# xionghuichen/mopo

Measured on AMD Instinct MI355X. Metric: model-rollout transitions/s (halfcheetah-mixed), higher is better.
Workload: dtype f32 (exact f32 operands: each split into 3 round-to-nearest bf16 parts with x0+x1+x2 == x for 2^-100 <= |x| < 2^127; 6 bf16 MFMA products, the 3 dropped ones <= 2^-23 |x w| in total; f32 accumulate; held to the fp32 parity tolerances); rollout actor: the same exact bf16x6 split; 1 GPU; C2 rollout: E=7 (5 elites), H=200 smv, obs=17, act=6, rollout_batch=50000 per GPU, horizon=5, penalty_coeff=1, learned-var penalty, env pool 101000 rows; rollout_batch_per_gpu=50000, horizon=5, parallelism=dp1

## Files before the change

### include/mopo_hip.h

```cpp
#ifndef MOPO_HIP_H
#define MOPO_HIP_H
#include <stdint.h>

#ifdef __cplusplus
extern "C" {
#endif

const char* mopo_last_error(void);
int mopo_version(void);

typedef struct mopo_bnn_s* mopo_bnn_t;

int mopo_bnn_create(mopo_bnn_t* out, int E, int obs_dim, int act_dim, int hidden, int smv, int dtype);
int mopo_bnn_device_hidden(int hidden, int dtype, int wide);
int mopo_bnn_destroy(mopo_bnn_t h);
int mopo_bnn_set_params(mopo_bnn_t h, const float* const* h_arrays, int n_arrays);
int mopo_bnn_predict(mopo_bnn_t h, const void* d_inputs, int inputs_f64, int64_t B,
                     float* d_mean, float* d_var, void* stream);
int64_t mopo_bnn_packed_bytes(mopo_bnn_t h);
int mopo_bnn_packed_copy(mopo_bnn_t h, int to_handle, void* d_buf, int64_t nbytes, void* stream);

enum { MOPO_TERM_NONE = 0, MOPO_TERM_HALFCHEETAH = 0, MOPO_TERM_WALKER2D = 1, MOPO_TERM_HOPPER = 2,
       MOPO_TERM_ANT = 3, MOPO_TERM_HUMANOID = 4, MOPO_TERM_KINDS = 5 };

typedef struct {
  const void* d_obs;
  int obs_f64;
  const float* d_act;
  int64_t B;
  const double* d_noise_sel;
  const int64_t* d_model_inds;
  int deterministic;
  float penalty_coeff;
  int penalty_learned_var;
  int term_kind;
  double* d_next_obs;
  double* d_rewards;
// ... 158 lines not shown
```

### mopo_amd/_lib.py

```python
import ctypes as C
import os

_HERE = os.path.dirname(os.path.abspath(__file__))
LIB_PATH = os.path.join(_HERE, 'libmopo_hip.so')

c_void_p, c_int, c_i64, c_u64, c_u32, c_float, c_double = (
    C.c_void_p, C.c_int, C.c_int64, C.c_uint64, C.c_uint32, C.c_float, C.c_double)


class FakeEnvArgs(C.Structure):
    _fields_ = [('d_obs', c_void_p), ('obs_f64', c_int), ('d_act', c_void_p), ('B', c_i64),
                ('d_noise_sel', c_void_p), ('d_model_inds', c_void_p), ('deterministic', c_int),
                ('penalty_coeff', c_float), ('penalty_learned_var', c_int), ('term_kind', c_int),
                ('d_next_obs', c_void_p), ('d_rewards', c_void_p), ('d_terminals', c_void_p),
                ('d_penalty', c_void_p), ('d_unpenalized', c_void_p), ('d_info_mean', c_void_p),
                ('d_info_std', c_void_p), ('d_log_prob', c_void_p), ('d_dev', c_void_p),
                ('d_ens_mean', c_void_p), ('d_ens_var', c_void_p)]


class PoolDesc(C.Structure):
    _fields_ = [('d_obs', c_void_p), ('d_act', c_void_p), ('d_rew', c_void_p), ('d_term', c_void_p),
                ('d_next_obs', c_void_p), ('d_state', c_void_p), ('max_size', c_i64)]


class RolloutArgs(C.Structure):
    _fields_ = [('d_env_obs', c_void_p), ('env_size', c_i64), ('d_start_idx', c_void_p),
                ('d_pi_params', c_void_p), ('pi_hidden', c_int), ('d_elites', c_void_p),
                ('n_elites', c_int), ('B', c_i64), ('horizon', c_int), ('penalty_coeff', c_float),
                ('term_kind', c_int), ('seed', c_u64), ('epoch', c_u32), ('uid_offset', c_i64),
                ('d_eps_act', c_void_p), ('d_eps_obs', c_void_p), ('d_model_inds', c_void_p),
                ('d_steps', c_void_p), ('penalty_learned_var', c_int), ('deterministic', c_int),
                ('rollout_random', c_int), ('d_act_uniform', c_void_p), ('actor_dtype', c_int)]


class EvalArgs(C.Structure):
    _fields_ = [('policy_deterministic', c_int), ('d_return', c_void_p), ('d_pen_return', c_void_p),
                ('d_pen_sum', c_void_p), ('d_length', c_void_p), ('d_terminated', c_void_p), ('d_stats', c_void_p)]


SIGNATURES = {
    'mopo_last_error': (C.c_char_p, []),
    'mopo_version': (c_int, []),
    'mopo_bnn_create': (c_int, [C.POINTER(c_void_p), c_int, c_int, c_int, c_int, c_int, c_int]),
    'mopo_bnn_destroy': (c_int, [c_void_p]),
    'mopo_bnn_set_params': (c_int, [c_void_p, C.POINTER(c_void_p), c_int]),
    'mopo_actor_device_hidden': (c_int, [c_int, c_int]),
    'mopo_bnn_device_hidden': (c_int, [c_int, c_int, c_int]),
    'mopo_bnn_predict': (c_int, [c_void_p, c_void_p, c_int, c_i64, c_void_p, c_void_p, c_void_p]),
    'mopo_bnn_packed_bytes': (c_i64, [c_void_p]),
    'mopo_bnn_packed_copy': (c_int, [c_void_p, c_int, c_void_p, c_i64, c_void_p]),
    'mopo_fakeenv_step': (c_int, [c_void_p, C.POINTER(FakeEnvArgs), c_void_p]),
    'mopo_sac_param_count': (c_i64, [c_int, c_int, c_int]),
    'mopo_actor_forward': (c_int, [c_void_p, c_int, c_int, c_int, c_void_p, c_int, c_i64, c_void_p,
                                   c_u64, c_u32, c_void_p, c_void_p, c_void_p]),
    'mopo_actor_forward_dtype': (c_int, [c_void_p, c_int, c_int, c_int, c_void_p, c_int, c_i64, c_void_p,
                                         c_u64, c_u32, c_void_p, c_void_p, c_int, c_void_p]),
    'mopo_pool_add': (c_int, [C.POINTER(PoolDesc), c_int, c_int, c_void_p, c_void_p, c_void_p, c_void_p,
                              c_void_p, c_i64, c_void_p]),
    'mopo_pool_gather': (c_int, [C.POINTER(PoolDesc), c_int, c_int, c_void_p, c_i64, c_void_p, c_void_p,
                                 c_void_p, c_void_p, c_void_p, c_i64, c_void_p]),
    'mopo_pool_random_indices': (c_int, [C.POINTER(PoolDesc), c_i64, c_u64, c_u32, c_void_p, c_void_p]),
    'mopo_pool_staged_block_bytes': (c_i64, [c_int, c_int, c_i64]),
    'mopo_pool_add_blocks': (c_int, [C.POINTER(PoolDesc), c_int, c_int, c_void_p, c_i64, c_int, c_i64, c_void_p,
                                     c_void_p]),
    'mopo_rollout_run_staged_steps': (c_int, [c_void_p, C.POINTER(RolloutArgs), C.POINTER(PoolDesc), c_int, c_int,
                                              c_void_p]),
    'mopo_bnn_train_create': (c_int, [C.POINTER(c_void_p), c_int, c_int, c_int, c_int, c_int, c_int, C.c_float]),
    'mopo_bnn_train_destroy': (c_int, [c_void_p]),
    'mopo_bnn_train_set_params': (c_int, [c_void_p, C.POINTER(c_void_p)]),
    'mopo_bnn_train_get_params': (c_int, [c_void_p, C.POINTER(c_void_p)]),
# ... 86 lines not shown
```

### mopo_amd/csrc/bnn_api.hip

```cpp
#include "mlp_tile.h"

#include <cmath>
#include <cstring>
#include <memory>
#include <string>
#include <vector>

using namespace mopo;

extern "C" int mopo_bnn_create(mopo_bnn_t* out, int E, int obs_dim, int act_dim, int hidden, int smv,
                               int dtype) {
  MOPO_REQUIRE(out != nullptr, "mopo_bnn_create: out is NULL");
  MOPO_REQUIRE(E >= 1 && E <= 256, "mopo_bnn_create: num_networks must be in [1, 256]");
  MOPO_REQUIRE(obs_dim >= 1 && act_dim >= 1, "mopo_bnn_create: bad obs/act dims");
  MOPO_REQUIRE(dtype >= 0 && dtype <= 4,
               "mopo_bnn_create: dtype must be 0 (fp32), 1 (bf16), 2 (bf16x3), 3 (bf16x6) or 4 (f16x3)");
  auto h = std::make_unique<Bnn>();
  h->E = E; h->O = obs_dim; h->A = act_dim; h->H = hidden; h->smv = smv; h->dtype = dtype;
  BnnDev& d = h->dev;
  d.E = E; d.O = obs_dim; d.A = act_dim; d.IN = obs_dim + act_dim; d.H = hidden; d.D = obs_dim + 1;
  if (d.IN > 16 * MAX_IN_KG || d.D > 32) {
    return fail("mopo_bnn_create: obs_dim + act_dim must be <= 64 and obs_dim <= 31 (got obs_dim " +
                std::to_string(obs_dim) + ", act_dim " + std::to_string(act_dim) + ")");
  }
// ... 14 lines not shown
  if (dtype == 3 && d.NB2 > 16) {
    return fail("mopo_bnn_create: bf16x6 supports hidden sizes <= 256 (use f16x3 or fp32)");
  }
  const int form = bnn_form_blocks(hidden, dtype, wide);
  if (form < 0) {
    if (dtype == DT_BF16 || dtype == DT_BF16X3)
      return fail("mopo_bnn_create: bf16 and bf16x3 run hidden sizes up to 64, 193..208 and 385..416 only (got " +
                  std::to_string(hidden) + "; fp32, bf16x6 and f16x3 run every hidden size up to 256)");
    return fail("mopo_bnn_create: no kernel for hidden size " + std::to_string(hidden) +
                " (every hidden size up to 256 runs in fp32, bf16x6 and f16x3, 385..400 in fp32 and f16x3; a wide "
                "model's bf16x6 / f16x3 stop at 208)");
  }
  h->HD = bnn_device_hidden(hidden, dtype, wide);
  d.NBH = form;
  d.NB2 = (d.NBH + 1) / 2 * 2;
  d.BS = d.NB2 * 16;
  *out = reinterpret_cast<mopo_bnn_t>(h.release());
  return 0;
}

extern "C" int mopo_bnn_device_hidden(int hidden, int dtype, int wide) {
  if (dtype < 0 || dtype > 4) return -1;
  return bnn_device_hidden(hidden, dtype, wide != 0);
}

extern "C" int mopo_bnn_destroy(mopo_bnn_t hh) {
  Bnn* h = reinterpret_cast<Bnn*>(hh);
  if (!h) return 0;
  if (h->buf) (void)hipFree(h->buf);
  if (h->bbuf) (void)hipFree(h->bbuf);
  delete h;
  return 0;
}

extern "C" int mopo_bnn_set_params(mopo_bnn_t hh, const float* const* arrs, int n) {
  Bnn* h = reinterpret_cast<Bnn*>(hh);
  MOPO_REQUIRE(h != nullptr, "mopo_bnn_set_params: NULL handle");
  MOPO_REQUIRE(n == (h->smv ? 16 : 14), "mopo_bnn_set_params: expected 16 (smv) or 14 arrays (.mat keys)");
  BnnDev& d = h->dev;
  const int E = h->E, IN = d.IN, H = h->H, D = d.D;
  const int KG0 = d.KG0, NBH = d.NBH, NBO = d.NBO;
  const int64_t hp = d.BS;
  const int64_t s_w0 = (int64_t)E * KG0 * NBH * 256, s_wh = 3LL * E * NBH * NBH * 256,
                s_whd = (int64_t)E * NBH * NBO * 256, s_b0 = E * hp, s_bh = 3 * E * hp,
                s_bhd = (int64_t)E * 3 * NBO * 16;
  const int64_t s_ws = (5LL * E + 63) / 64 * 64;
// ... 54 lines not shown
  }
  if (rc == 0) rc = pack(head.data(), head.size(), whd, H, 2 * D, NBH, NBO, 2);
  if (rc) return rc;
  {
    std::vector<float> aux((size_t)s_bhd, 0.f);
    for (int e = 0; e < E; ++e) {
      float* x = aux.data() + (size_t)e * 3 * NBO * 16;
      for (int sl = 0; sl < NBO * 16; ++sl) {
        const int c = head_col(sl, D);
        if (c < 0) continue;
        x[sl] = headb[(size_t)e * 2 * D + c];
        if (c >= D) {
          x[NBO * 16 + sl] = arrs[h->smv ? 14 : 12][c - D];
          x[2 * NBO * 16 + sl] = arrs[h->smv ? 15 : 13][c - D];
        }
      }
    }
    MOPO_HIP(hipMemcpy(bhd, aux.data(), aux.size() * sizeof(float), hipMemcpyHostToDevice));
  }
  if (h->dtype != 0 && rc == 0) {
    const int NB2 = d.NB2, KG = NB2 / 2, P = bf16_parts(h->dtype), KG0B = (KG0 + 1) / 2;
    const bool kpack = bnn_kpack(h->dtype, NB2, NBH, h->HD);
    const int64_t SLM = kpack ? (KG - 1) * P + 1 : KG * P;
    const int64_t f0 = (int64_t)E * KG0B * P * NB2, fh = 3LL * E * SLM * NB2, fd = (int64_t)E * SLM * NBO;
    if (!h->bbuf) MOPO_HIP(hipMalloc(&h->bbuf, (f0 + fh + fd) * 256 * sizeof(float)));
    h->bbuf_bytes = (f0 + fh + fd) * 256 * (int64_t)sizeof(float);
    float* b0f = reinterpret_cast<float*>(h->bbuf);
    float* bhf = b0f + f0 * 256;
    float* bdf = bhf + fh * 256;
    std::vector<float> scale_h(5 * E), inv_h(5 * E, 1.f);
    float* scale_d = nullptr;
    DevFree scale_guard{scale_d};
    if (h->dtype == DT_F16X3) MOPO_HIP(hipMalloc(&scale_d, E * sizeof(float)));
    auto member_scales = [&](const float* src, int K, int N, int layer) {
      for (int e = 0; e < E; ++e) {
        float m = 0.f;
        for (int64_t i = 0; i < (int64_t)K * N; ++i) m = std::max(m, std::fabs(src[(int64_t)e * K * N + i]));
        int ex = 0;
        if (m > 0.f && std::isfinite(m)) std::frexp(m, &ex);
        const int k = m > 0.f && std::isfinite(m) ? 15 - ex : 0;
        scale_h[layer * E + e] = std::ldexp(1.f, k);
        inv_h[layer * E + e] = std::ldexp(1.f, -k);
      }
    };
    int layer_idx = 0;
    auto packh = [&](const float* src, size_t nsrc, float* dst, int K, int N, int KGb, int NB, int perm_n,
                     bool pk = false) -> int {
      MOPO_HIP(hipMemcpy(stage, src, nsrc * sizeof(float), hipMemcpyHostToDevice));
      const int64_t mstride = (pk ? SLM : (int64_t)KGb * P) * NB;
      if (pk) {
        if (pack_frags_kpack(stage, (short*)dst, E, K, N, KGb, NB, perm_n, mstride, 0)) return -1;
        --KGb;
      }
      if (h->dtype == DT_F16X3) {
        member_scales(src, K, N, layer_idx);
        MOPO_HIP(hipMemcpy(scale_d, scale_h.data() + layer_idx * E, E * sizeof(float), hipMemcpyHostToDevice));
      }
      if (pack_frags16(stage, (short*)dst, E, K, N, KGb, NB, perm_n, P, h->dtype == DT_F16X3 ? scale_d : nullptr, mstride, 0))
        return -1;
      MOPO_HIP(hipDeviceSynchronize());
      ++layer_idx;
      return 0;
    };
    if (rc == 0) rc = packh(W[0], (size_t)E * IN * H, b0f, IN, H, KG0B, NB2, 1);
    for (int l = 0; l < 3 && rc == 0; ++l)
      rc = packh(W[1 + l], (size_t)E * H * H, bhf + (int64_t)l * E * SLM * NB2 * 256, H, H, KG, NB2, 1, kpack);
    if (rc == 0) rc = packh(head.data(), head.size(), bdf, H, 2 * D, KG, NBO, 2, kpack);
    if (rc == 0 && h->dtype == DT_F16X3)
      rc = hipMemcpy(wsc, inv_h.data(), 5 * E * sizeof(float), hipMemcpyHostToDevice) == hipSuccess ? 0
                                                                                                 : fail("bnn: scale copy");
    d.w0b = b0f; d.whb = bhf; d.whdb = bdf; d.wscale = wsc;
  }
  if (rc) return -1;
  MOPO_HIP(hipMemcpy(mu, arrs[0], IN * sizeof(float), hipMemcpyHostToDevice));
  MOPO_HIP(hipMemcpy(sg, arrs[1], IN * sizeof(float), hipMemcpyHostToDevice));
  MOPO_HIP(hipMemcpy(mx, maxlv, D * sizeof(float), hipMemcpyHostToDevice));
  MOPO_HIP(hipMemcpy(mn, minlv, D * sizeof(float), hipMemcpyHostToDevice));
  d.w0 = w0; d.wh = wh; d.whd = whd; d.b0 = b0; d.bh = bh; d.bhd = bhd;
  d.mu = mu; d.sigma = sg; d.maxlv = mx; d.minlv = mn;
  h->has_params = true;
  return 0;
}

extern "C" int mopo_bnn_predict(mopo_bnn_t hh, const void* x, int x_f64, int64_t B, float* mean,
                                float* var, void* stream) {
  Bnn* h = reinterpret_cast<Bnn*>(hh);
  MOPO_REQUIRE(h != nullptr, "mopo_bnn_predict: NULL handle");
  MOPO_REQUIRE(B >= 0 && B < (1LL << 31) / 32, "mopo_bnn_predict: batch too large");
  if (B == 0) return 0;
  MOPO_REQUIRE(x && mean && var, "mopo_bnn_predict: NULL pointer");
// ... 34 lines not shown
```

### mopo_amd/csrc/bnn_kernels.h

```cpp
#pragma once
#include "mlp_tile.h"

#include <type_traits>

#ifndef BNN_KPB
#define BNN_KPB 1
#endif
#ifndef BNN_MINB_WIDE
#define BNN_MINB_WIDE 2
#endif
#ifndef BNN_R13
#define BNN_R13 1
#endif
#ifndef BNN_FWD_WAVES
#define BNN_FWD_WAVES 4
#endif
#ifndef BNN_SPLIT_HOLD_F32
#define BNN_SPLIT_HOLD_F32 1
#endif
#ifndef BNN_SPLIT_MINB
#define BNN_SPLIT_MINB 3
#endif
#ifndef BNN_SPLIT_WAVES
#define BNN_SPLIT_WAVES 4
// ... 596 lines not shown
    layer2(w.whb + ((int64_t)l * E + e) * KG * P * NB2 * 256, hf, std::integral_constant<int, KG>{},
           w.bh + ((int64_t)l * E + e) * bs);
    to_input(lds_bias, inv_row * w.wscale[(1 + l) * E + e]);
  }
  f32x4 hd[NBO];
  layer_lds_split_f32<KG, NBO, WAVES, SLOT, P, 1, true, NBO, KH>(w.whdb + (int64_t)e * KG * P * NBO * 256, hf, hd,
                                                                 lds, wv, lane, s_in);
  const float f = inv_row * w.wscale[4 * E + e] * kNegLn2;
#pragma unroll
  for (int nb = 0; nb < NBO; ++nb) hd[nb] *= f;
  int lane_e;
  asm volatile("v_mbcnt_lo_u32_b32 %0, -1, 0\n\tv_mbcnt_hi_u32_b32 %0, -1, %0" : "=v"(lane_e));
  const int64_t row_e = (int64_t)((grp * WAVES + __builtin_amdgcn_readfirstlane(wv)) * 16 + (lane_e & 15));
  const bool ok_e = row_e < count;
  head_epilogue<NBO, MODE>(w, a, hd, e, row_e, count, g, w.bhd + (int64_t)e * 3 * NBO * 16,
                           (MODE == FWD_ROLLOUT && a.sel && ok_e) ? a.sel[row_e] : -1);
}

template <int NB2, int P, int WAVES>
constexpr int ring_minb() {
  const int b = (P == 3 ? (NB2 == 16 ? BNN_RING_MINB_X6_16 : BNN_RING_MINB_X6) : BNN_RING_MINB) * 4 / WAVES;
  return b > 0 ? b : 1;
}
template <int NB2, int NBO, int MODE, int WAVES, int P, int DEPTH, int NBU = NB2, int KG0B = 1, bool KP = false>
__global__ __launch_bounds__(WAVES * 64, (ring_minb<NB2, P, WAVES>())) void bnn_fwd_ring_kernel(const BnnDev w, const FwdArgs a) {
  static_assert(P == 1 || P == 2 || P == 3, "1: bf16, 2: f16x3, 3: bf16x6 (the exact 3-part bf16 split)");
  static_assert(DEPTH >= 3, "ring of at least 3 slots");
  constexpr bool F16 = P == 2;
  constexpr bool RBUF = true;
  constexpr int HPS = BNN_RING_HEAD_MERGE && Stage<P * NBO, WAVES>::SLOTS <= Stage<NB2, WAVES>::SLOTS ? P : 1;
  constexpr int P0 = P * KG0B;
  constexpr bool KH = NBU < NB2;
  static_assert(!KP || (P == 3 && KH), "the packed remainder is the 3-part split's, behind an odd block count");
  constexpr int KG = NB2 / 2, KGF = KP ? KG - 1 : KG;
  constexpr int SLH = KGF * P + KP, SLD = KGF * (P / HPS) + KP;
  constexpr int NS = P0 + 3 * SLH + SLD;
  constexpr int JHEAD = P0 + 3 * SLH;
  constexpr int SLOT = Stage<(NB2 > HPS * NBO ? NB2 : HPS * NBO), WAVES>::SLOTS * 256;
  constexpr int BIAS_LDS = (NB2 * 4 + 63) / 64 * 256;
  __shared__ __attribute__((aligned(16))) float lds[DEPTH * SLOT + 2 * BIAS_LDS];
  float* lds_bias0 = lds + DEPTH * SLOT;
  const int lane = threadIdx.x & 63, wv = __builtin_amdgcn_readfirstlane(threadIdx.x >> 6), m = lane & 15, g = lane >> 4;
  const int64_t count = a.d_count ? (int64_t)*a.d_count : a.B;
  const int groups = ceil_div(a.ntiles, WAVES);
  const int C = ceil_div(groups, 8);
  const int xcd = blockIdx.x & 7, jb = blockIdx.x >> 3;
  const int e = __builtin_amdgcn_readfirstlane(jb / C), grp = __builtin_amdgcn_readfirstlane(xcd * C + jb % C);
  if (grp >= groups) return;
  const int64_t row = (int64_t)(grp * WAVES + wv) * 16 + m;
  if ((int64_t)grp * WAVES * 16 >= count) return;
  const int IN = w.IN, O = w.O, E = w.E;
  const bool ok = row < count;
  auto row_max = [&](float mx) {
    mx = fmaxf(mx, __shfl_xor(mx, 16));
    return fmaxf(mx, __shfl_xor(mx, 32));
  };
// ... 60 lines not shown
    row_scale(row_max(mx0), s_in, inv_row);
  }
  wait_vm_lgkm0<0>();
  __builtin_amdgcn_sched_barrier(0);
  stage_bias<NB2 * 4, WAVES, RBUF>(w.b0 + e * bs, lds_bias0, wv, lane);
  RingRun<0, DEPTH - 1>::run([&](auto jc) { issue(jc); });

  constexpr float kNegLog2e = -1.4426950408889634f, kNegLn2 = -0.6931471805599453f;
  f32x4 acc[NB2 > NBO ? NB2 : NBO];
  float hf[KG][8];
  bf16x8 cur[P];
  const float* lds_bias = lds_bias0;
  auto bias4 = [&](int off) { return __builtin_bit_cast(f32x4, *reinterpret_cast<const bf16x8*>(lds_bias + off)); };
  constexpr bool DEF = BNN_F16Q_DEFER;
  constexpr bool FOLD = F16 && DEF && BNN_F16_FOLD;
  auto to_input = [&](float f) {
    float mx = 0.f;
#pragma unroll
    for (int c = 0; c < KG; ++c) {
      const f32x4 b0 = bias4((2 * c) * 16 + 4 * g);
      const f32x4 b1 = bias4((2 * c + 1) * 16 + 4 * g);
#pragma unroll
      for (int t = 0; t < 4; ++t) {
        const float u0 = fmaf(acc[2 * c][t], f, b0[t]);
        const float u1 = 2 * c + 1 < NBU ? fmaf(acc[2 * c + 1][t], f, b1[t]) : 0.f;
        hf[c][t] = DEF ? u0 : swish_log2(u0);
        hf[c][4 + t] = DEF || 2 * c + 1 >= NBU ? u1 : swish_log2(u1);
        if constexpr (F16) mx = fmaxf(mx, fmaxf(fabsf(hf[c][t]), fabsf(hf[c][4 + t])));
      }
    }
    if constexpr (F16) row_scale(row_max(mx), s_in, inv_row);
  };
  auto act = [&](int c, int j) {
    if ((j < 4 || 2 * c + 1 < NBU) && !(KP && c == KG - 1 && j >= 2)) {
      const float u = hf[c][j];
      hf[c][j] = FOLD ? u * __builtin_amdgcn_rcpf(fmaf(__builtin_amdgcn_exp2f(u), inv_row, inv_row)) : swish_log2(u);
    }
  };
  auto parts = [&](const float (&v)[8], auto prescaled, auto half) {
    if constexpr (F16) {
      u32x4v h4, l4;
#pragma unroll
      for (int q = 0; q < 4; ++q) {
        if (decltype(half)::value && q >= 2) {
          h4[q] = l4[q] = 0u;
          continue;
        }
// ... 27 lines not shown
  };
  auto parts_rem = [&](const float (&v)[8]) {
    if constexpr (P == 3) {
      uint32_t pr[3];
      split_bf16_pair<3>(v[0], v[1], pr);
      u32x4v bf, bh;
#pragma unroll
      for (int d = 0; d < 4; ++d) {
        bf[d] = pr[kpack_slot(2 * d).xp];
        bh[d] = d < 2 ? pr[kpack_slot(d < 2 ? 8 + 2 * d : 8).xp] : 0u;
      }
      cur[0] = __builtin_bit_cast(bf16x8, bf);
      cur[1] = __builtin_bit_cast(bf16x8, bh);
    }
  };
  auto layer = [&](auto Lc, auto& in) {
    constexpr int L = decltype(Lc)::value;
    constexpr int KGL = L == 0 ? KG0B : KG, NBL = L == 4 ? NBO : NB2, NBUL = L == 4 ? NBO : NBU;
    constexpr bool KHL = L > 0 && KH;
    constexpr bool DEFER = DEF && L > 0;
    constexpr int J0 = L == 0 ? 0 : P0 + SLH * (L - 1);
    constexpr int PPS = L == 4 ? HPS : 1, SPK = P / PPS;
    constexpr bool KPL = KP && L > 0;
    constexpr int SLL = SPK * (KPL ? KGL - 1 : KGL) + KPL;
    static_assert(SLL == (L == 0 ? P0 : L == 4 ? SLD : SLH), "the layer's share of the slice stream");
#pragma unroll
    for (int nb = 0; nb < NBL; ++nb) acc[nb] = zero4();
    if constexpr (DEFER) {
#pragma unroll
      for (int j = 0; j < 8; ++j) act(0, j);
    }
    RingRun<J0, J0 + SLL>::run([&](auto jc) {
      constexpr int J = decltype(jc)::value, s = J - J0;
      constexpr bool REM = KPL && s == SLL - 1;
      constexpr int kg = REM ? KGL - 1 : s / SPK, p0 = REM ? 0 : (s % SPK) * PPS;
      if constexpr (REM)
        parts_rem(in[kg]);
      else if constexpr (p0 == 0)
        parts(in[kg], std::integral_constant<bool, FOLD && (L > 0)>{}, std::integral_constant<bool, KHL && kg + 1 == KGL>{});
      constexpr int N = [] {
        int n = 0;
        for (int i = 1; i <= DEPTH - 2; ++i) {
          const int Jx = J + i;
          const int nf = Jx < JHEAD ? NB2 : (KP && Jx == NS - 1 ? NBO : HPS * NBO);
          n += Jx >= NS ? 0 : (nf + WAVES - 1) / WAVES;
        }
// ... 1 lines not shown
      }();
      wait_vm_lgkm0<N>();
      __builtin_amdgcn_s_barrier();
      if constexpr (s == 0 && L < 3)
        stage_bias<NB2 * 4, WAVES, RBUF>(w.bh + ((int64_t)L * E + e) * bs, lds_bias0 + ((L + 1) & 1) * BIAS_LDS, wv, lane);
      issue(std::integral_constant<int, J + DEPTH - 1>{});
      __builtin_amdgcn_sched_barrier(0);
      const float* b = lds + (J % DEPTH) * SLOT;
      auto frag = [&](int i) { return *reinterpret_cast<const bf16x8*>(b + (((i / NBUL) * NBL + i % NBUL) * 64 + lane) * 4); };
      constexpr int PF = P == 3 ? (NB2 == 16 ? BNN_RING_PF_X6_16 : BNN_RING_PF_X6) : BNN_RING_PF, NFR = REM ? NBUL : PPS * NBUL;
      bf16x8 fq[PF];
#pragma unroll
      for (int k = 0; k < PF; ++k)
        if (k < NFR) fq[k] = frag(k);
#pragma unroll
      for (int i = 0; i < NFR; ++i) {
        const int p = p0 + i / NBUL, nb = i % NBUL;
        const bf16x8 fr = fq[i % PF];
        if (i + PF < NFR) fq[i % PF] = frag(i + PF);
        if constexpr (BNN_RING_PIN) __builtin_amdgcn_sched_barrier(0x0406);
        if constexpr (REM) {
          acc[nb] = mfma_16x16x32<F16>(fr, cur[0], acc[nb]);
          acc[nb] = mfma_16x16x32<F16>(fr, cur[1], acc[nb]);
        } else {
#pragma unroll
          for (int q = P - 1 - p; q >= 0; --q)
            acc[nb] = (KHL && kg + 1 == KGL) ? mfma_16x16x16_lo<F16>(fr, cur[q], acc[nb])
                                             : mfma_16x16x32<F16>(fr, cur[q], acc[nb]);
        }
        if constexpr (DEFER && kg + 1 < KGL) {
          constexpr int V = (8 + P - 1) / P;
#pragma unroll
          for (int v = 0; v < V; ++v)
            if (V * p + v < 8 && nb == ((v + 1) * NBUL / V - 1 > 0 ? (v + 1) * NBUL / V - 1 : 0)) act(kg + 1, V * p + v);
        }
      }
    });
  };
  {
    float x1[KG0B][8];
#pragma unroll
    for (int c = 0; c < KG0B; ++c)
#pragma unroll
      for (int j = 0; j < 8; ++j) x1[c][j] = xv[c][j];
    layer(std::integral_constant<int, 0>{}, x1);
  }
  to_input(inv_row * wsc[0] * kNegLog2e);
  layer(std::integral_constant<int, 1>{}, hf);
  lds_bias = lds_bias0 + BIAS_LDS;
  to_input(inv_row * wsc[1]);
  layer(std::integral_constant<int, 2>{}, hf);
  lds_bias = lds_bias0;
  to_input(inv_row * wsc[2]);
  layer(std::integral_constant<int, 3>{}, hf);
  lds_bias = lds_bias0 + BIAS_LDS;
  to_input(inv_row * wsc[3]);
  layer(std::integral_constant<int, 4>{}, hf);
  f32x4 hd[NBO];
  const float f = inv_row * wsc[4] * kNegLn2;
#pragma unroll
  for (int nb = 0; nb < NBO; ++nb) hd[nb] = acc[nb] * f;
  int lane_e;
  asm volatile("v_mbcnt_lo_u32_b32 %0, -1, 0\n\tv_mbcnt_hi_u32_b32 %0, -1, %0" : "=v"(lane_e));
  const int64_t row_e = (int64_t)(grp * WAVES + wv) * 16 + (lane_e & 15);
  const bool ok_e = row_e < count;
  head_epilogue<NBO, MODE>(w, a, hd, e, row_e, count, g, w.bhd + (int64_t)e * 3 * NBO * 16,
                           (MODE == FWD_ROLLOUT && a.sel && ok_e) ? a.sel[row_e] : -1);
}

template <class F>
static inline void with_mode(int mode, F&& f) {
  if (mode == FWD_PREDICT) f(std::integral_constant<int, FWD_PREDICT>{});
  else f(std::integral_constant<int, FWD_ROLLOUT>{});
}

template <int NB2, int NBO, int P, int DEPTH, int KG0B = 1, bool KP = false>
static int launch_ring(const Bnn* h, int mode, FwdArgs a, hipStream_t s) {
  constexpr int WV = BNN_RING_WAVES;
  a.ntiles = (int)ceil_div((int)a.B, 16);
  if (a.ntiles == 0) return 0;
  dim3 grid(8 * ceil_div(ceil_div(a.ntiles, WV), 8) * h->E), block(64 * WV);
  constexpr int NBU = NB2 == 14 ? NB2 - 1 : NB2;
  with_mode(mode, [&](auto m) {
    hipLaunchKernelGGL((bnn_fwd_ring_kernel<NB2, NBO, decltype(m)::value, WV, P, DEPTH, NBU, KG0B, KP>), grid, block, 0, s,
                       h->dev, a);
  });
  MOPO_HIP(hipGetLastError());
  return 0;
}
template <int NB2>
static bool ring_shape(const Bnn* h) { return NB2 <= 16 && (NB2 == 14 ? h->dev.NBH == 13 : h->dev.NBH == NB2); }
static inline bool kpack_shape(const Bnn* h) { return bnn_kpack(h->dtype, h->dev.NB2, h->dev.NBH, h->HD); }
template <int NB2, int NBO, int KG0B = 1>
static int launch_ring_x6(const Bnn* h, int mode, const FwdArgs& a, hipStream_t s) {
  if constexpr (NB2 == 14)
    if (kpack_shape(h)) return launch_ring<NB2, NBO, 3, BNN_RING_DEPTH_BF16, KG0B, true>(h, mode, a, s);
  if (kpack_shape(h)) return fail("bnn bf16x6: packed-remainder weights at a shape without the packed kernel");
  return launch_ring<NB2, NBO, 3, BNN_RING_DEPTH_BF16, KG0B>(h, mode, a, s);
}

constexpr int FWD_WAVES = BNN_FWD_WAVES;

template <int KG0, int NBH, int NBO, int R, int TQ0 = 4, int TQH = 4>
static int launch_fwd_t(const Bnn* h, int mode, FwdArgs a, hipStream_t s) {
  a.ntiles = (int)ceil_div((int)a.B, 16 * R);
  if (a.ntiles == 0) return 0;
  dim3 grid(ceil_div(a.ntiles, FWD_WAVES) * h->E), block(64 * FWD_WAVES);
  with_mode(mode, [&](auto m) {
    hipLaunchKernelGGL((bnn_fwd_kernel<KG0, NBH, NBO, R, decltype(m)::value, FWD_WAVES, TQ0, TQH>), grid, block, 0, s,
                       h->dev, a);
  });
  MOPO_HIP(hipGetLastError());
  return 0;
}

}
```

### mopo_amd/csrc/bnn_pack.h

```cpp
#pragma once
#include "mlp_tile.h"

#include <algorithm>

namespace mopo {

__global__ void pack_frags_kernel(const float* __restrict__ src, float* __restrict__ dst, int E, int K,
                                  int N, int KG, int NB, int perm_k, int perm_n) {
  int64_t total = (int64_t)E * KG * NB * 256;
  for (int64_t i = blockIdx.x * (int64_t)blockDim.x + threadIdx.x; i < total;
       i += (int64_t)gridDim.x * blockDim.x) {
    int t = i & 3, lane = (i >> 2) & 63;
    int64_t f = i >> 8;
    int nb = f % NB;
    int kg = (f / NB) % KG;
    int e = f / ((int64_t)NB * KG);
    int k = kg * 16 + 4 * (lane >> 4) + t, n = nb * 16 + (lane & 15);
    if (perm_k) k = slot_feat(k, K);
    if (perm_n == 1) n = slot_feat(n, N);
    else if (perm_n == 2) n = head_col(n, N / 2);
    dst[i] = (k >= 0 && n >= 0 && k < K && n < N) ? src[((int64_t)e * K + k) * N + n] : 0.f;
  }
}

// ... 26 lines not shown
__global__ void pack_frags_kpack_kernel(const float* __restrict__ src, short* __restrict__ dst, int E, int K, int N,
                                        int KG, int NB, int perm_n, int64_t mstride) {
  int64_t total = (int64_t)E * NB * 512;
  for (int64_t i = blockIdx.x * (int64_t)blockDim.x + threadIdx.x; i < total;
       i += (int64_t)gridDim.x * blockDim.x) {
    int j = i & 7, lane = (i >> 3) & 63;
    int64_t f = i >> 9;
    int nb = f % NB;
    int e = f / NB;
    const KPackSlot sl = kpack_slot(j);
    int k = slot_feat((KG - 1) * 32 + bf16_kperm(lane >> 4, sl.k), K), n = nb * 16 + (lane & 15);
    if (perm_n == 1) n = slot_feat(n, N);
    else if (perm_n == 2) n = head_col(n, N / 2);
    short parts[3];
    split_bf16<3>((k >= 0 && n >= 0 && k < K && n < N) ? src[((int64_t)e * K + k) * N + n] : 0.f, parts);
    short v = parts[0];
#pragma unroll
    for (int q = 1; q < 3; ++q)
      if (q == sl.wp) v = parts[q];
    dst[(e * mstride + (int64_t)(KG - 1) * 3 * NB + nb) * 512 + (i & 511)] = v;
  }
}

__global__ void pack_frags_f16s_kernel(const float* __restrict__ src, short* __restrict__ dst, int E, int K, int N,
                                       int KG, int NB, int perm_k, int perm_n, const float* __restrict__ scale) {
  constexpr int P = 2;
  int64_t total = (int64_t)E * KG * P * NB * 512;
  for (int64_t i = blockIdx.x * (int64_t)blockDim.x + threadIdx.x; i < total;
       i += (int64_t)gridDim.x * blockDim.x) {
    int j = i & 7, lane = (i >> 3) & 63;
    int64_t f = i >> 9;
    int nb = f % NB;
    int p = (f / NB) % P;
    int kg = (f / ((int64_t)NB * P)) % KG;
    int e = f / ((int64_t)NB * P * KG);
    int k = kg * 32 + bf16_kperm(lane >> 4, j), n = nb * 16 + (lane & 15);
    if (perm_k) k = slot_feat(k, K);
    if (perm_n == 1) n = slot_feat(n, N);
    else if (perm_n == 2) n = head_col(n, N / 2);
    const F16Parts q = split_f16_scaled((k >= 0 && n >= 0 && k < K && n < N) ? src[((int64_t)e * K + k) * N + n] : 0.f,
                                        scale[e]);
    dst[i] = p == 0 ? q.hi : q.lo;
  }
}

__global__ void pack_bias_kernel(const float* __restrict__ src, float* __restrict__ dst, int E, int N,
// ... 19 lines not shown
  MOPO_HIP(hipGetLastError());
  return 0;
}

int pack_frags16(const float* src, short* dst, int E, int K, int N, int KG, int NB, int perm_n, int P,
                 const float* scale, int64_t mstride, hipStream_t s) {
  const dim3 grid = pack_grid((int64_t)E * KG * P * NB * 512), block(256);
  if (scale) hipLaunchKernelGGL(pack_frags_f16s_kernel, grid, block, 0, s, src, dst, E, K, N, KG, NB, 1, perm_n, scale);
  else if (P == 3) hipLaunchKernelGGL(pack_frags_bf16_kernel<3>, grid, block, 0, s, src, dst, E, K, N, KG, NB, 1, perm_n, mstride);
  else if (P == 2) hipLaunchKernelGGL(pack_frags_bf16_kernel<2>, grid, block, 0, s, src, dst, E, K, N, KG, NB, 1, perm_n, mstride);
  else hipLaunchKernelGGL(pack_frags_bf16_kernel<1>, grid, block, 0, s, src, dst, E, K, N, KG, NB, 1, perm_n, mstride);
  MOPO_HIP(hipGetLastError());
  return 0;
}

int pack_frags_kpack(const float* src, short* dst, int E, int K, int N, int KG, int NB, int perm_n, int64_t mstride,
                     hipStream_t s) {
  hipLaunchKernelGGL(pack_frags_kpack_kernel, pack_grid((int64_t)E * NB * 512), dim3(256), 0, s, src, dst, E, K, N, KG, NB,
                     perm_n, mstride);
  MOPO_HIP(hipGetLastError());
  return 0;
}

}
```

### mopo_amd/csrc/internal.h

```cpp
#pragma once
#include "common.h"
#include "../../include/mopo_hip.h"

namespace mopo {

constexpr int MAX_IN_KG = 4;
__host__ __device__ constexpr bool bnn_wide(int IN, int D) { return IN > 32 || D > 24; }

struct BnnDev {
  int E, O, A, IN, H, D;
  int KG0, NBH, NBO;
  const float* w0;
  const float* wh;
  const float* whd;
  const float* b0;
  const float* bh;
  const float* bhd;
  const float* mu;
  const float* sigma;
  const float* maxlv;
  const float* minlv;
  int BS;
  int NB2;
  const float* w0b;
  const float* whb;
  const float* whdb;
  const float* wscale;
};

enum { DT_FP32 = 0, DT_BF16 = 1, DT_BF16X3 = 2, DT_BF16X6 = 3, DT_F16X3 = 4 };
__host__ __device__ constexpr int bf16_parts(int dtype) { return dtype < 1 ? 1 : (dtype == DT_F16X3 ? 2 : dtype); }

__host__ __device__ constexpr int tail_steps(int F) { return (F & 15) == 0 ? 4 : ((F & 15) + 3) >> 2; }

__host__ __device__ constexpr bool bnn_kpack(int dtype, int NB2, int NBH, int H) {
  return dtype == DT_BF16X6 && NB2 == 14 && NBH == 13 && tail_steps(H) == 2;
}

inline int bnn_form_blocks(int hidden, int dtype, bool wide) {
  if (hidden < 1) return -1;
  const int nb = (hidden + 15) / 16;
  const bool split = dtype == 3  || dtype == 4 ;
  if (!wide && dtype != 0) {
    if (dtype != 4 && (nb == 1 || nb == 3)) return nb;
    if (dtype != 3 && nb == 26) return nb;
    if (!split) return (nb == 2 || nb == 4 || nb == 13 || nb == 25) ? nb : -1;
  }
  if (wide && dtype != 0 && !split) return -1;
  const int forms[6] = {2, 4, 8, 13, 16, 25};
  const int top = dtype == 0 ? 25 : (wide ? 13 : (dtype == 3 ? 16 : 25));
  for (int f : forms)
    if (f >= nb && f <= top) return (f == 25 && nb < 25) ? -1 : f;
  return -1;
}
inline int bnn_device_hidden(int hidden, int dtype, bool wide) {
  const int f = bnn_form_blocks(hidden, dtype, wide);
  if (f < 0) return -1;
  const int lo = (f == 8 || f == 16) ? 16 * f : 16 * (f - 1) + 1;
  return hidden > lo ? hidden : lo;
// ... 35 lines not shown
  int ntiles;
  int xcd_members;
  float* mean;
  float* var;
  uint32_t* pen_bits;
  const int32_t* sel;
  float* mean_sel;
  float* std_sel;
  float* mean_all;
  float* std_all;
  int64_t all_stride;
};

int launch_bnn_fwd(const Bnn* h, int mode, const FwdArgs& a, hipStream_t s);
int launch_bnn_fwd_widths(const Bnn* h, int mode, const FwdArgs& a, hipStream_t s);
int launch_bnn_fwd_widths16(const Bnn* h, int mode, const FwdArgs& a, hipStream_t s);
int pack_frags(const float* src, float* dst, int E, int K, int N, int KG, int NB, hipStream_t s, int perm_k = 0,
               int perm_n = 0);
int pack_bias(const float* src, float* dst, int E, int N, int NP, float mul, hipStream_t s);
int pack_frags16(const float* src, short* dst, int E, int K, int N, int KG, int NB, int perm_n, int P,
                 const float* scale, int64_t mstride, hipStream_t s);
int pack_frags_kpack(const float* src, short* dst, int E, int K, int N, int KG, int NB, int perm_n, int64_t mstride,
                     hipStream_t s);

template <class F>
__device__ __forceinline__ bool term_fn_at(int kind, const F& nobs, int O) {
  if (kind == MOPO_TERM_WALKER2D) {
    double hh = nobs(0), an = nobs(1);
    bool not_done = (hh > 0.8) && (hh < 2.0) && (an > -1.0) && (an < 1.0);
    return !not_done;
  }
  if (kind == MOPO_TERM_HOPPER) {
    bool fin = true, small = true;
    for (int d = 0; d < O; ++d) {
      double v = nobs(d);
      fin = fin && isfinite(v);
      if (d >= 1) small = small && (v < 100.0);
    }
    double hh = nobs(0), an = nobs(1);
    bool not_done = fin && small && (hh > 0.7) && (fabs(an) < 0.2);
    return !not_done;
  }
  if (kind == MOPO_TERM_ANT) {
    bool fin = true;
    for (int d = 0; d < O; ++d) fin = fin && isfinite(nobs(d));
    double x = nobs(0);
// ... 16 lines not shown
```

### mopo_amd/csrc/mlp_tile.h

```cpp
#pragma once
#include <type_traits>

#include "internal.h"

namespace mopo {

__host__ __device__ __forceinline__ int slot_feat(int slot, int F) {
  const int blk = slot >> 4, rem = F - 16 * blk;
  if (rem >= 16) return slot;
  if (rem <= 0) return -1;
  const int q = (rem + 3) >> 2, g = (slot >> 2) & 3, t = slot & 3, f = q * g + t;
  return (t < q && f < rem) ? 16 * blk + f : -1;
}

__host__ __device__ __forceinline__ int head_col(int slot, int D) {
  const int nb = slot >> 4, g = (slot >> 2) & 3, t = slot & 3, j = 4 * nb + t, Q = (D + 3) >> 2;
  if (j < Q) return g + 4 * j < D ? D + g + 4 * j : -1;
  if (j < 2 * Q) return g + 4 * (j - Q) < D ? g + 4 * (j - Q) : -1;
  return -1;
}


typedef __attribute__((address_space(3))) void* lds_void_t;

// ... 242 lines not shown

struct KPackSlot {
  int k, xp, wp;
};
constexpr int KPACK_SLOTS = 12;
__host__ __device__ constexpr KPackSlot kpack_slot(int i) {
  constexpr int XP[6] = {0, 0, 0, 1, 2, 1}, WP[6] = {0, 1, 2, 0, 0, 1};
  return {i & 1, XP[i >> 1], WP[i >> 1]};
}
constexpr bool kpack_table_ok() {
  for (int k = 0; k < 2; ++k)
    for (int p = 0; p < 3; ++p)
      for (int q = 0; q < 3; ++q) {
        int n = 0;
        for (int i = 0; i < KPACK_SLOTS; ++i) n += kpack_slot(i).k == k && kpack_slot(i).xp == p && kpack_slot(i).wp == q;
        if (n != (p + q < 3 ? 1 : 0)) return false;
      }
  for (int i = 8; i < KPACK_SLOTS; ++i)
    if (kpack_slot(i).wp != kpack_slot(i - 8).wp) return false;
  return true;
}
static_assert(kpack_table_ok(), "every product (p, q), p + q < 3, exactly once per k, and no other");

template <int KG, int NB, int WAVES, int SLOT, int P, int PS = P, bool F16 = false, int NBU = NB, bool KH = false>
__device__ __forceinline__ void layer_lds_split(const float* __restrict__ wf, const bf16x8 (&in)[P][KG],
                                                f32x4 (&acc)[NB], float* lds, int w, int lane,
                                                const float* __restrict__ bias = nullptr, float* lds_bias = nullptr) {
  static_assert(P % PS == 0, "parts per slice must divide the parts");
  constexpr int SPK = P / PS, S = KG * SPK, NF = PS * NB;
  static_assert(Stage<NF, WAVES>::SLOTS * 256 <= SLOT, "slice larger than its buffer");
#pragma unroll
  for (int nb = 0; nb < NB; ++nb) acc[nb] = zero4();
  __syncthreads();
  stage_slice<NF, WAVES>(wf, lds, w, lane);
  if (bias) stage_bias<NB * 4, WAVES>(bias, lds_bias, w, lane);
#pragma unroll
  for (int s = 0; s < S; ++s) {
    __syncthreads();
    if (s + 1 < S) stage_slice<NF, WAVES>(wf + (s + 1) * NF * 256, lds + ((s + 1) & 1) * SLOT, w, lane);
    __builtin_amdgcn_sched_barrier(0);
    const int kg = s / SPK;
    const float* b = lds + (s & 1) * SLOT;
#ifndef BNN_SPLIT_NOPF
    bf16x8 fr_next = *reinterpret_cast<const bf16x8*>(b + lane * 4);
#endif
#pragma unroll
// ... 173 lines not shown
```

Baseline: 102.2 million transitions/s.

## Pack the half-used last output block's split products into fewer MFMAs

For the bf16x6 ring kernel at the 13-block hidden shape, the last output column block only uses half its columns. The half-empty column slots now carry different weight parts of the same columns, so each k-slice issues fewer MFMAs for that block, and the two halves are summed afterwards. This needs a new weight-packing kernel, an mpack mode template parameter, and zeroing of the padded outputs. The aim is to cut wasted matrix-core work on padding columns, at the cost of a more intricate packing scheme that must still produce each split product exactly once.

```diff
diff --git a/include/mopo_hip.h b/include/mopo_hip.h
--- a/include/mopo_hip.h
+++ b/include/mopo_hip.h
@@ -13,6 +13,7 @@
 
 int mopo_bnn_create(mopo_bnn_t* out, int E, int obs_dim, int act_dim, int hidden, int smv, int dtype);
 int mopo_bnn_device_hidden(int hidden, int dtype, int wide);
+int mopo_bnn_mpack(int hidden, int dtype, int obs_dim, int act_dim);
 int mopo_bnn_destroy(mopo_bnn_t h);
 int mopo_bnn_set_params(mopo_bnn_t h, const float* const* h_arrays, int n_arrays);
 int mopo_bnn_predict(mopo_bnn_t h, const void* d_inputs, int inputs_f64, int64_t B,
diff --git a/mopo_amd/_lib.py b/mopo_amd/_lib.py
--- a/mopo_amd/_lib.py
+++ b/mopo_amd/_lib.py
@@ -46,6 +46,7 @@
     'mopo_bnn_set_params': (c_int, [c_void_p, C.POINTER(c_void_p), c_int]),
     'mopo_actor_device_hidden': (c_int, [c_int, c_int]),
     'mopo_bnn_device_hidden': (c_int, [c_int, c_int, c_int]),
+    'mopo_bnn_mpack': (c_int, [c_int, c_int, c_int, c_int]),
     'mopo_bnn_predict': (c_int, [c_void_p, c_void_p, c_int, c_i64, c_void_p, c_void_p, c_void_p]),
     'mopo_bnn_packed_bytes': (c_i64, [c_void_p]),
     'mopo_bnn_packed_copy': (c_int, [c_void_p, c_int, c_void_p, c_i64, c_void_p]),
diff --git a/mopo_amd/csrc/bnn_api.hip b/mopo_amd/csrc/bnn_api.hip
--- a/mopo_amd/csrc/bnn_api.hip
+++ b/mopo_amd/csrc/bnn_api.hip
@@ -60,6 +60,16 @@
 extern "C" int mopo_bnn_device_hidden(int hidden, int dtype, int wide) {
   if (dtype < 0 || dtype > 4) return -1;
   return bnn_device_hidden(hidden, dtype, wide != 0);
+}
+
+extern "C" int mopo_bnn_mpack(int hidden, int dtype, int obs_dim, int act_dim) {
+  if (dtype < 0 || dtype > 4 || obs_dim < 1 || act_dim < 0) return -1;
+  const int IN = obs_dim + act_dim, D = obs_dim + 1;
+  if (IN > 16 * MAX_IN_KG || D > 32) return -1;
+  const bool wide = bnn_wide(IN, D);
+  const int NBH = bnn_form_blocks(hidden, dtype, wide);
+  if (NBH < 0) return -1;
+  return bnn_mpack(dtype, (NBH + 1) / 2 * 2, NBH, bnn_device_hidden(hidden, dtype, wide), D, wide ? 4 : ceil_div(2 * D, 16));
 }
 
 extern "C" int mopo_bnn_destroy(mopo_bnn_t hh) {
@@ -160,6 +170,7 @@
     const int NB2 = d.NB2, KG = NB2 / 2, P = bf16_parts(h->dtype), KG0B = (KG0 + 1) / 2;
     const bool kpack = bnn_kpack(h->dtype, NB2, NBH, h->HD);
     const int64_t SLM = kpack ? (KG - 1) * P + 1 : KG * P;
+    const int mpack = bnn_mpack(h->dtype, NB2, NBH, h->HD, D, NBO);
     const int64_t f0 = (int64_t)E * KG0B * P * NB2, fh = 3LL * E * SLM * NB2, fd = (int64_t)E * SLM * NBO;
     if (!h->bbuf) MOPO_HIP(hipMalloc(&h->bbuf, (f0 + fh + fd) * 256 * sizeof(float)));
     h->bbuf_bytes = (f0 + fh + fd) * 256 * (int64_t)sizeof(float);
@@ -183,7 +194,7 @@
     };
     int layer_idx = 0;
     auto packh = [&](const float* src, size_t nsrc, float* dst, int K, int N, int KGb, int NB, int perm_n,
-                     bool pk = false) -> int {
+                     bool pk = false, int mpb = -1) -> int {
       MOPO_HIP(hipMemcpy(stage, src, nsrc * sizeof(float), hipMemcpyHostToDevice));
       const int64_t mstride = (pk ? SLM : (int64_t)KGb * P) * NB;
       if (pk) {
@@ -196,14 +207,16 @@
       }
       if (pack_frags16(stage, (short*)dst, E, K, N, KGb, NB, perm_n, P, h->dtype == DT_F16X3 ? scale_d : nullptr, mstride, 0))
         return -1;
+      if (mpb >= 0 && pack_frags_mpack(stage, (short*)dst, E, K, N, KGb, NB, mpb, perm_n, mstride, 0)) return -1;
       MOPO_HIP(hipDeviceSynchronize());
       ++layer_idx;
       return 0;
     };
-    if (rc == 0) rc = packh(W[0], (size_t)E * IN * H, b0f, IN, H, KG0B, NB2, 1);
+    const int mpb = mpack ? NBH - 1 : -1, mpbd = mpack == 2 ? NBO - 1 : -1;
+    if (rc == 0) rc = packh(W[0], (size_t)E * IN * H, b0f, IN, H, KG0B, NB2, 1, false, mpb);
     for (int l = 0; l < 3 && rc == 0; ++l)
-      rc = packh(W[1 + l], (size_t)E * H * H, bhf + (int64_t)l * E * SLM * NB2 * 256, H, H, KG, NB2, 1, kpack);
-    if (rc == 0) rc = packh(head.data(), head.size(), bdf, H, 2 * D, KG, NBO, 2, kpack);
+      rc = packh(W[1 + l], (size_t)E * H * H, bhf + (int64_t)l * E * SLM * NB2 * 256, H, H, KG, NB2, 1, kpack, mpb);
+    if (rc == 0) rc = packh(head.data(), head.size(), bdf, H, 2 * D, KG, NBO, 2, kpack, mpbd);
     if (rc == 0 && h->dtype == DT_F16X3)
       rc = hipMemcpy(wsc, inv_h.data(), 5 * E * sizeof(float), hipMemcpyHostToDevice) == hipSuccess ? 0
                                                                                                  : fail("bnn: scale copy");
diff --git a/mopo_amd/csrc/bnn_kernels.h b/mopo_amd/csrc/bnn_kernels.h
--- a/mopo_amd/csrc/bnn_kernels.h
+++ b/mopo_amd/csrc/bnn_kernels.h
@@ -642,7 +642,7 @@
   const int b = (P == 3 ? (NB2 == 16 ? BNN_RING_MINB_X6_16 : BNN_RING_MINB_X6) : BNN_RING_MINB) * 4 / WAVES;
   return b > 0 ? b : 1;
 }
-template <int NB2, int NBO, int MODE, int WAVES, int P, int DEPTH, int NBU = NB2, int KG0B = 1, bool KP = false>
+template <int NB2, int NBO, int MODE, int WAVES, int P, int DEPTH, int NBU = NB2, int KG0B = 1, bool KP = false, int MP = 0>
 __global__ __launch_bounds__(WAVES * 64, (ring_minb<NB2, P, WAVES>())) void bnn_fwd_ring_kernel(const BnnDev w, const FwdArgs a) {
   static_assert(P == 1 || P == 2 || P == 3, "1: bf16, 2: f16x3, 3: bf16x6 (the exact 3-part bf16 split)");
   static_assert(DEPTH >= 3, "ring of at least 3 slots");
@@ -652,6 +652,7 @@
   constexpr int P0 = P * KG0B;
   constexpr bool KH = NBU < NB2;
   static_assert(!KP || (P == 3 && KH), "the packed remainder is the 3-part split's, behind an odd block count");
+  static_assert(MP == 0 || ((MP == 1 || MP == 2) && KP), "the packed output block comes with the packed remainder");
   constexpr int KG = NB2 / 2, KGF = KP ? KG - 1 : KG;
   constexpr int SLH = KGF * P + KP, SLD = KGF * (P / HPS) + KP;
   constexpr int NS = P0 + 3 * SLH + SLD;
@@ -758,7 +759,7 @@
       const f32x4 b1 = bias4((2 * c + 1) * 16 + 4 * g);
 #pragma unroll
       for (int t = 0; t < 4; ++t) {
-        const float u0 = fmaf(acc[2 * c][t], f, b0[t]);
+        const float u0 = MP && 2 * c == NBU - 1 && t >= 2 ? 0.f : fmaf(acc[2 * c][t], f, b0[t]);
         const float u1 = 2 * c + 1 < NBU ? fmaf(acc[2 * c + 1][t], f, b1[t]) : 0.f;
         hf[c][t] = DEF ? u0 : swish_log2(u0);
         hf[c][4 + t] = DEF || 2 * c + 1 >= NBU ? u1 : swish_log2(u1);
@@ -832,6 +833,7 @@
     constexpr int J0 = L == 0 ? 0 : P0 + SLH * (L - 1);
     constexpr int PPS = L == 4 ? HPS : 1, SPK = P / PPS;
     constexpr bool KPL = KP && L > 0;
+    constexpr int MPB = MP == 0 ? -1 : (L < 4 ? NBU - 1 : (MP == 2 ? NBO - 1 : -1));
     constexpr int SLL = SPK * (KPL ? KGL - 1 : KGL) + KPL;
     static_assert(SLL == (L == 0 ? P0 : L == 4 ? SLD : SLH), "the layer's share of the slice stream");
 #pragma unroll
@@ -879,6 +881,10 @@
         if constexpr (REM) {
           acc[nb] = mfma_16x16x32<F16>(fr, cur[0], acc[nb]);
           acc[nb] = mfma_16x16x32<F16>(fr, cur[1], acc[nb]);
+        } else if (MPB >= 0 && nb == MPB) {
+#pragma unroll
+          for (int q = P - 1; q >= 0; --q)
+            if ((mpack_xparts(p) >> q) & 1) acc[nb] = mfma_16x16x32<F16>(fr, cur[q], acc[nb]);
         } else {
 #pragma unroll
           for (int q = P - 1 - p; q >= 0; --q)
@@ -893,6 +899,10 @@
         }
       }
     });
+    if constexpr (MPB >= 0) {
+      acc[MPB][0] += acc[MPB][2];
+      acc[MPB][1] += acc[MPB][3];
+    }
   };
   {
     float x1[KG0B][8];
@@ -931,7 +941,7 @@
   else f(std::integral_constant<int, FWD_ROLLOUT>{});
 }
 
-template <int NB2, int NBO, int P, int DEPTH, int KG0B = 1, bool KP = false>
+template <int NB2, int NBO, int P, int DEPTH, int KG0B = 1, bool KP = false, int MP = 0>
 static int launch_ring(const Bnn* h, int mode, FwdArgs a, hipStream_t s) {
   constexpr int WV = BNN_RING_WAVES;
   a.ntiles = (int)ceil_div((int)a.B, 16);
@@ -939,7 +949,7 @@
   dim3 grid(8 * ceil_div(ceil_div(a.ntiles, WV), 8) * h->E), block(64 * WV);
   constexpr int NBU = NB2 == 14 ? NB2 - 1 : NB2;
   with_mode(mode, [&](auto m) {
-    hipLaunchKernelGGL((bnn_fwd_ring_kernel<NB2, NBO, decltype(m)::value, WV, P, DEPTH, NBU, KG0B, KP>), grid, block, 0, s,
+    hipLaunchKernelGGL((bnn_fwd_ring_kernel<NB2, NBO, decltype(m)::value, WV, P, DEPTH, NBU, KG0B, KP, MP>), grid, block, 0, s,
                        h->dev, a);
   });
   MOPO_HIP(hipGetLastError());
@@ -948,11 +958,21 @@
 template <int NB2>
 static bool ring_shape(const Bnn* h) { return NB2 <= 16 && (NB2 == 14 ? h->dev.NBH == 13 : h->dev.NBH == NB2); }
 static inline bool kpack_shape(const Bnn* h) { return bnn_kpack(h->dtype, h->dev.NB2, h->dev.NBH, h->HD); }
+static inline int mpack_shape(const Bnn* h) {
+  return bnn_mpack(h->dtype, h->dev.NB2, h->dev.NBH, h->HD, h->dev.D, h->dev.NBO);
+}
 template <int NB2, int NBO, int KG0B = 1>
 static int launch_ring_x6(const Bnn* h, int mode, const FwdArgs& a, hipStream_t s) {
   if constexpr (NB2 == 14)
-    if (kpack_shape(h)) return launch_ring<NB2, NBO, 3, BNN_RING_DEPTH_BF16, KG0B, true>(h, mode, a, s);
-  if (kpack_shape(h)) return fail("bnn bf16x6: packed-remainder weights at a shape without the packed kernel");
+    if (kpack_shape(h) && h->dev.NBO == NBO) {
+      switch (mpack_shape(h)) {
+        case 1: return launch_ring<NB2, NBO, 3, BNN_RING_DEPTH_BF16, KG0B, true, 1>(h, mode, a, s);
+        case 2: return launch_ring<NB2, NBO, 3, BNN_RING_DEPTH_BF16, KG0B, true, 2>(h, mode, a, s);
+      }
+      return fail("bnn bf16x6: packed-remainder weights without the packed output block");
+    }
+  if (kpack_shape(h) || mpack_shape(h))
+    return fail("bnn bf16x6: packed-remainder weights at a shape without the packed kernel");
   return launch_ring<NB2, NBO, 3, BNN_RING_DEPTH_BF16, KG0B>(h, mode, a, s);
 }
 
diff --git a/mopo_amd/csrc/bnn_pack.h b/mopo_amd/csrc/bnn_pack.h
--- a/mopo_amd/csrc/bnn_pack.h
+++ b/mopo_amd/csrc/bnn_pack.h
@@ -72,6 +72,31 @@
   }
 }
 
+__global__ void pack_frags_mpack_kernel(const float* __restrict__ src, short* __restrict__ dst, int E, int K, int N,
+                                        int KGF, int NB, int nb, int perm_n, int64_t mstride) {
+  int64_t total = (int64_t)E * KGF * 3 * 512;
+  for (int64_t i = blockIdx.x * (int64_t)blockDim.x + threadIdx.x; i < total;
+       i += (int64_t)gridDim.x * blockDim.x) {
+    int j = i & 7, lane = (i >> 3) & 63;
+    int64_t f = i >> 9;
+    int p = f % 3;
+    int kg = (f / 3) % KGF;
+    int e = f / (3 * (int64_t)KGF);
+    const int r = lane & 15, t = r & 3;
+    int k = slot_feat(kg * 32 + bf16_kperm(lane >> 4, j), K), n = nb * 16 + (r & ~2);
+    if (perm_n == 1) n = slot_feat(n, N);
+    else if (perm_n == 2) n = head_col(n, N / 2);
+    short parts[3];
+    split_bf16<3>((k >= 0 && n >= 0 && k < K && n < N) ? src[((int64_t)e * K + k) * N + n] : 0.f, parts);
+    const int wp = mpack_wpart(p, t);
+    short v = 0;
+#pragma unroll
+    for (int q = 0; q < 3; ++q)
+      if (q == wp) v = parts[q];
+    dst[(e * mstride + (int64_t)(kg * 3 + p) * NB + nb) * 512 + (i & 511)] = v;
+  }
+}
+
 __global__ void pack_frags_f16s_kernel(const float* __restrict__ src, short* __restrict__ dst, int E, int K, int N,
                                        int KG, int NB, int perm_k, int perm_n, const float* __restrict__ scale) {
   constexpr int P = 2;
@@ -137,4 +162,12 @@
   return 0;
 }
 
+int pack_frags_mpack(const float* src, short* dst, int E, int K, int N, int KGF, int NB, int nb, int perm_n,
+                     int64_t mstride, hipStream_t s) {
+  hipLaunchKernelGGL(pack_frags_mpack_kernel, pack_grid((int64_t)E * KGF * 3 * 512), dim3(256), 0, s, src, dst, E, K, N,
+                     KGF, NB, nb, perm_n, mstride);
+  MOPO_HIP(hipGetLastError());
+  return 0;
 }
+
+}
diff --git a/mopo_amd/csrc/internal.h b/mopo_amd/csrc/internal.h
--- a/mopo_amd/csrc/internal.h
+++ b/mopo_amd/csrc/internal.h
@@ -35,6 +35,11 @@
 
 __host__ __device__ constexpr bool bnn_kpack(int dtype, int NB2, int NBH, int H) {
   return dtype == DT_BF16X6 && NB2 == 14 && NBH == 13 && tail_steps(H) == 2;
+}
+
+__host__ __device__ constexpr int bnn_mpack(int dtype, int NB2, int NBH, int H, int D, int NBO) {
+  if (!bnn_kpack(dtype, NB2, NBH, H)) return 0;
+  return 2 * ((D + 3) >> 2) == 4 * (NBO - 1) + 2 ? 2 : 1;
 }
 
 inline int bnn_form_blocks(int hidden, int dtype, bool wide) {
@@ -116,6 +121,8 @@
                  const float* scale, int64_t mstride, hipStream_t s);
 int pack_frags_kpack(const float* src, short* dst, int E, int K, int N, int KG, int NB, int perm_n, int64_t mstride,
                      hipStream_t s);
+int pack_frags_mpack(const float* src, short* dst, int E, int K, int N, int KGF, int NB, int nb, int perm_n,
+                     int64_t mstride, hipStream_t s);
 
 template <class F>
 __device__ __forceinline__ bool term_fn_at(int kind, const F& nobs, int O) {
diff --git a/mopo_amd/csrc/mlp_tile.h b/mopo_amd/csrc/mlp_tile.h
--- a/mopo_amd/csrc/mlp_tile.h
+++ b/mopo_amd/csrc/mlp_tile.h
@@ -288,6 +288,24 @@
 }
 static_assert(kpack_table_ok(), "every product (p, q), p + q < 3, exactly once per k, and no other");
 
+__host__ __device__ constexpr int mpack_wpart(int p, int t) {
+  return t < 2 ? (p == 1 ? 2 : 0) : (p == 0 ? 1 : -1);
+}
+__host__ __device__ constexpr int mpack_xparts(int p) { return p == 0 ? 0b011 : (p == 1 ? 0b001 : 0b100); }
+constexpr bool mpack_table_ok() {
+  for (int xp = 0; xp < 3; ++xp)
+    for (int wp = 0; wp < 3; ++wp) {
+      int n = 0;
+      for (int p = 0; p < 3; ++p)
+        for (int half = 0; half < 2; ++half) n += ((mpack_xparts(p) >> xp) & 1) && mpack_wpart(p, 2 * half) == wp;
+      if (n != (xp + wp < 3 ? 1 : 0)) return false;
+    }
+  for (int p = 0; p < 3; ++p)
+    if (mpack_wpart(p, 0) != mpack_wpart(p, 1) || mpack_wpart(p, 2) != mpack_wpart(p, 3)) return false;
+  return true;
+}
+static_assert(mpack_table_ok(), "every product (p, q), p + q < 3, exactly once per slot, and no other");
+
 template <int KG, int NB, int WAVES, int SLOT, int P, int PS = P, bool F16 = false, int NBU = NB, bool KH = false>
 __device__ __forceinline__ void layer_lds_split(const float* __restrict__ wf, const bf16x8 (&in)[P][KG],
                                                 f32x4 (&acc)[NB], float* lds, int w, int lane,
```

After: 102.6 million transitions/s (median of 6 runs). About the same (+0.4%).
